# ypw0102/GDR

Hardware: AMD Instinct MI355X
Metric: queries/sec on NQ-320k (768-d) (higher is better)
Workload: dtype f32; 1 GPU; C2/ragged/prefilter: t5-base encoder 512 q/GPU + Q.D^T top-100, 320000x768 corpus; batch_per_gpu=512, global_batch=512, seq_len=40, corpus_rows=320000, dim=768, k=100, encoder_rows=ragged

## Files before the change

gdr_amd/_ffi.py:

```python
import ctypes as C
import os

_HERE = os.path.dirname(os.path.abspath(__file__))
LIB_PATH = os.environ.get("GDR_HIP_LIB") or os.path.join(_HERE, "libgdr_hip.so")

GDR_OK, GDR_EINVAL, GDR_ENOSPC, GDR_EHIP = 0, -1, -2, -3
ABI_VERSION = 9
RERANK_POSITIONS = 1
SIM_EXHAUSTIVE = 1
SIM_NO_STREAM = 2
EPI_NONE, EPI_RESIDUAL, EPI_RELU, EPI_BIAS, EPI_BIAS_RELU, EPI_BIAS_RESIDUAL, EPI_BIAS_GELU = range(7)


class GdrError(RuntimeError):
    pass


class GdrT5Dims(C.Structure):
    _fields_ = [("vocab_size", C.c_int32), ("d_model", C.c_int32), ("d_kv", C.c_int32), ("d_ff", C.c_int32),
                ("num_heads", C.c_int32), ("num_layers", C.c_int32), ("rel_buckets", C.c_int32),
                ("rel_max_distance", C.c_int32), ("eps", C.c_float)]


class GdrT5EncLayer(C.Structure):
    _fields_ = [(n, C.c_void_p) for n in ("ln_attn", "wqkv", "wo", "ln_ff", "wi", "wo_ff")]


class GdrT5EncoderWeights(C.Structure):
    _fields_ = [("dims", GdrT5Dims), ("embed", C.c_void_p), ("rel_bias", C.c_void_p), ("final_ln", C.c_void_p),
                ("layers", C.POINTER(GdrT5EncLayer))]


class GdrBertLayer(C.Structure):
    _fields_ = [(n, C.c_void_p) for n in ("wqkv", "bqkv", "wo", "bo", "ln1_w", "ln1_b", "wi", "bi", "wo2", "bo2", "ln2_w",
                                          "ln2_b")]


class GdrBertWeights(C.Structure):
    _fields_ = [("vocab_size", C.c_int32), ("d_model", C.c_int32), ("num_heads", C.c_int32), ("d_ff", C.c_int32),
                ("num_layers", C.c_int32), ("max_pos", C.c_int32), ("type_vocab", C.c_int32), ("eps", C.c_float),
                ("word_emb", C.c_void_p), ("pos_emb", C.c_void_p), ("type_emb", C.c_void_p), ("emb_ln_w", C.c_void_p),
                ("emb_ln_b", C.c_void_p), ("layers", C.POINTER(GdrBertLayer))]


class GdrTrie(C.Structure):
    _fields_ = [("child", C.c_void_p), ("eos_ok", C.c_void_p), ("n_nodes", C.c_int32), ("V", C.c_int32)]


class GdrPrefixTable(C.Structure):
    _fields_ = [("child", C.c_void_p), ("n_nodes", C.c_int32), ("V", C.c_int32), ("n_table", C.c_int32),
                ("kv", C.c_void_p), ("W", C.c_void_p), ("complete_levels", C.c_int32)]


class GdrClusterIndex(C.Structure):
    _fields_ = [("n_clusters", C.c_int32), ("key_len", C.c_int32), ("table_size", C.c_int32), ("slots", C.c_void_p),
                ("keys", C.c_void_p), ("key_lens", C.c_void_p), ("offsets", C.c_void_p), ("members", C.c_void_p)]


class GdrT5DecLayer(C.Structure):
    _fields_ = [(n, C.c_void_p) for n in ("ln_self", "wqkv", "wo", "ln_cross", "wq_c", "wkv_c", "wo_c", "ln_ff", "wi",
                                          "wo_ff")]


class GdrAdaptorLayer(C.Structure):
    _fields_ = [(n, C.c_void_p) for n in ("in_w", "in_b", "out_w", "out_b", "ln1_w", "ln1_b", "cross_const", "ln2_w",
                                          "ln2_b", "lin1_w", "lin1_b", "lin2_w", "lin2_b", "ln3_w", "ln3_b")]


class GdrT5DecoderWeights(C.Structure):
    _fields_ = [("dims", GdrT5Dims), ("out_vocab", C.c_int32), ("max_out_len", C.c_int32),
                ("adaptor_layers", C.c_int32), ("adaptor_nhead", C.c_int32), ("adaptor_ff", C.c_int32),
                ("adaptor_eps", C.c_float), ("dec_embed", C.c_void_p), ("self_rel_bias", C.c_void_p),
                ("cross_rel_bias", C.c_void_p), ("final_ln", C.c_void_p), ("layers", C.POINTER(GdrT5DecLayer)),
                ("alayers", C.POINTER(GdrAdaptorLayer)), ("head_w", C.c_void_p), ("head_e", C.c_void_p)]


_vp, _i, _i64, _sz, _f = C.c_void_p, C.c_int, C.c_int64, C.c_size_t, C.c_float
SIGNATURES = {
    "gdr_last_error": (C.c_char_p, []),
    "gdr_abi_version": (_i, []),
    "gdr_device_fault_pending": (_i, []),
    "gdr_device_fault_clear": (None, []),
    "gdr_device_fault_inject_for_tests": (None, []),
# ... 128 lines not shown
```

gdr_amd/csrc/encoder.hip:

```cpp
#include <stdlib.h>

#include "layers.h"

namespace gdr {

constexpr size_t ENC_SPLITK_BYTES = (size_t)112 << 20;
static_assert(STREAMK_BYTES <= ENC_SPLITK_BYTES, "stream-K scratch must fit the split-K region");

static int enc_streamk(char* splitk_region, StreamK* sk, hipStream_t stream) {
  sk->part = reinterpret_cast<float*>(splitk_region);
  sk->flag = reinterpret_cast<int32_t*>(splitk_region + STREAMK_PART_BYTES);
  sk->epoch = 0;
  if (hipMemsetAsync(sk->flag, 0, 512 * sizeof(int32_t), stream) != hipSuccess) {
    set_error("t5_encoder: memset of the stream-K flags failed");
    return GDR_EHIP;
  }
  return GDR_OK;
}

struct EncWs {
  size_t off_h, off_nx, off_qkv, off_ctx, off_ff, off_splitk, off_bf, total;
};

static EncWs enc_ws(const GdrT5Dims& dm, int64_t M, bool bf16 = false) {
  EncWs w{};
  const size_t inner = (size_t)dm.num_heads * dm.d_kv;
  size_t o = 0;
  w.off_h = o, o += align_up((size_t)M * dm.d_model * 4, 256);
  w.off_nx = o, o += align_up((size_t)M * dm.d_model * 4, 256);
  w.off_qkv = o, o += align_up((size_t)M * 3 * inner * 4, 256);
  w.off_ctx = o, o += align_up((size_t)M * inner * 4, 256);
  w.off_ff = o, o += align_up((size_t)M * dm.d_ff * 4, 256);
  w.off_splitk = o, o += ENC_SPLITK_BYTES;
  w.off_bf = o;
  if (bf16) o += align_up((size_t)M * (dm.d_ff > dm.d_model ? dm.d_ff : dm.d_model) * 2, 256);
  w.total = o;
  return w;
}

}

extern "C" size_t gdr_t5_encoder_workspace_bytes(const GdrT5Dims* dims, int B, int L) {
  if (!dims || B <= 0 || L <= 0) return 0;
  return gdr::enc_ws(*dims, (int64_t)B * L).total;
}

namespace gdr {
static int t5_encoder_impl(const GdrT5EncoderWeights* w, const int64_t* ids, const int64_t* mask, int B, int L,
                           float* out_hidden, float* out_pooled, void* workspace, size_t workspace_bytes, bool bf16,
                           hipStream_t stream) {
  if (B == 0) return GDR_OK;
  GDR_CHECK_ARG(w && ids && out_hidden && workspace, "t5_encoder: null pointer");
  const GdrT5Dims& dm = w->dims;
  GDR_CHECK_ARG(B > 0 && L > 0 && L <= 128, "t5_encoder: B=%d L=%d (L must be in [1,128])", B, L);
  GDR_CHECK_ARG(dm.d_model % 4 == 0 && dm.d_kv % 4 == 0 && dm.d_ff % 4 == 0, "t5_encoder: dims must be multiples of 4");
  GDR_CHECK_ARG(w->embed && w->rel_bias && w->final_ln && w->layers, "t5_encoder: null weight pointer");
  const int64_t M = (int64_t)B * L;
  const EncWs ws = enc_ws(dm, M, bf16);
  GDR_CHECK_ARG(!bf16 || (dm.d_model % 8 == 0 && dm.d_ff % 8 == 0 && (dm.num_heads * dm.d_kv) % 8 == 0),
                "t5_encoder_bf16: dims must be multiples of 8");
// ... 197 lines not shown
    const bool pooled_only = out_hidden == nullptr;
    for (int i = 0; i < dm.num_layers; ++i) {
      const GdrT5EncLayer& ly = w->layers[i];
      GDR_CHECK_ARG(ly.ln_attn && ly.wqkv && ly.wo && ly.ln_ff && ly.wi && ly.wo_ff, "t5_encoder_ragged: layer %d null weight", i);
      if ((rc = launch_rmsnorm_bf16_dev(h, ly.ln_attn, abf, rows_dev, M, d, dm.eps, stream))) return rc;
      if ((rc = lin16(abf, ly.wqkv, qkv, 3 * inner, M, rows_dev, 3 * inner, d, 0, nullptr, 1))) return rc;
      if ((rc = launch_attention(at, stream))) return rc;
      if (pooled_only && i == dm.num_layers - 1) {
        if ((rc = launch_gather_rows(static_cast<const float*>(abf), seq_off, B, inner / 2, static_cast<float*>(ctx_cls16), stream)))
          return rc;
        if ((rc = launch_gather_rows(h, seq_off, B, d, h_cls, stream))) return rc;
        if ((rc = lin16(ctx_cls16, ly.wo, h_cls, d, B, nullptr, d, inner, 0, h_cls, 0))) return rc;
        if ((rc = launch_rmsnorm_bf16(h_cls, ly.ln_ff, nx_cls16, B, d, dm.eps, stream))) return rc;
        if ((rc = lin16(nx_cls16, ly.wi, static_cast<float*>(ff_cls16), dm.d_ff, B, nullptr, dm.d_ff, d, 1, nullptr, 1))) return rc;
        if ((rc = lin16(ff_cls16, ly.wo_ff, h_cls, d, B, nullptr, d, dm.d_ff, 0, h_cls, 0))) return rc;
        return launch_rmsnorm(h_cls, w->final_ln, out_pooled, B, d, dm.eps, nullptr, 1, stream);
      }
      if ((rc = lin16(abf, ly.wo, h, d, M, rows_dev, d, inner, 0, h, 0))) return rc;
      if ((rc = launch_rmsnorm_bf16_dev(h, ly.ln_ff, abf, rows_dev, M, d, dm.eps, stream))) return rc;
      if ((rc = lin16(abf, ly.wi, ff, dm.d_ff, M, rows_dev, dm.d_ff, d, 1, nullptr, 1))) return rc;
      if ((rc = lin16(ff, ly.wo_ff, h, d, M, rows_dev, d, dm.d_ff, 0, h, 0))) return rc;
    }
    if ((rc = launch_rmsnorm_dev(h, w->final_ln, nx, rows_dev, M, d, dm.eps, stream))) return rc;
    if (out_pooled && (rc = launch_gather_rows(nx, seq_off, B, d, out_pooled, stream))) return rc;
    if (out_hidden) {
      if (hipMemsetAsync(out_hidden, 0, (size_t)M * d * sizeof(float), stream) != hipSuccess) {
        set_error("t5_encoder_ragged: memset failed");
        return GDR_EHIP;
      }
      if ((rc = launch_scatter_rows(nx, row_src, rows_dev, M, d, out_hidden, stream))) return rc;
    }
    return GDR_OK;
  }
  float* h = reinterpret_cast<float*>(base + ws.off_h);
  float* nx = reinterpret_cast<float*>(base + ws.off_nx);
  float* qkv = reinterpret_cast<float*>(base + ws.off_qkv);
  float* ctx = reinterpret_cast<float*>(base + ws.off_ctx);
  float* ff = reinterpret_cast<float*>(base + ws.off_ff);
  float* ctx_cls = reinterpret_cast<float*>(base + rw.ctx_cls);
  float* h_cls = reinterpret_cast<float*>(base + rw.h_cls);
  float* nx_cls = reinterpret_cast<float*>(base + rw.nx_cls);
  float* ff_cls = reinterpret_cast<float*>(base + rw.ff_cls);
  StreamK sk{};
  if ((rc = enc_streamk(base + ws.off_splitk, &sk, stream))) return rc;
  float* skw = reinterpret_cast<float*>(base + ws.off_splitk);
  auto linear = [&](const float* A, int64_t lda, const float* W, float* C, int64_t ldc, int N, int K, int epi,
                    const float* residual) -> int {
    if (small)
      return launch_linear_f32_ws(A, lda, W, K, C, ldc, M, N, K, epi, nullptr, residual, ldc, skw, ENC_SPLITK_BYTES, stream, &sk,
                                  rows_dev, live_rows_hint);
    return launch_linear_f32_dev(A, lda, W, K, C, ldc, M, rows_dev, N, K, epi, nullptr, residual, ldc, live_rows_hint, stream,
                                 &sk);
  };
  if ((rc = launch_embed_packed(w->embed, ids, row_src, rows_dev, M, d, dm.vocab_size, h, stream))) return rc;

  AttnArgs at{};
  at.q = qkv, at.k = qkv + inner, at.v = qkv + 2 * inner, at.out = ctx;
  at.ldq = at.ldk = at.ldv = 3 * inner, at.ldo = inner;
  at.q_bstride = at.k_bstride = at.o_bstride = L;
  at.B = B, at.H = H, at.dk = dk, at.Lq = L, at.Lk = L;
  at.q_pos0 = 0, at.scale = 1.0f;
  at.rel_bias = w->rel_bias, at.bidirectional = 1, at.num_buckets = dm.rel_buckets;
  at.lut = make_bucket_lut(dm.rel_buckets / 2, dm.rel_max_distance);
  at.key_mask = mask, at.mask_bstride = L, at.causal = 0, at.causal_neg_inf = 0;
  at.kv_rows = nullptr, at.kv_group = 1;
  at.seq_off = seq_off, at.seq_len = seq_len;

  const bool pooled_only = out_hidden == nullptr && big;
  for (int i = 0; i < dm.num_layers; ++i) {
    const GdrT5EncLayer& ly = w->layers[i];
    GDR_CHECK_ARG(ly.ln_attn && ly.wqkv && ly.wo && ly.ln_ff && ly.wi && ly.wo_ff, "t5_encoder_ragged: layer %d null weight", i);
    if ((rc = launch_rmsnorm_dev(h, ly.ln_attn, nx, rows_dev, M, d, dm.eps, stream))) return rc;
    if ((rc = linear(nx, d, ly.wqkv, qkv, 3 * inner, 3 * inner, d, GDR_EPI_NONE, nullptr))) return rc;
    if ((rc = launch_attention(at, stream))) return rc;
    if (pooled_only && i == dm.num_layers - 1) {
      if ((rc = launch_gather_rows(ctx, seq_off, B, inner, ctx_cls, stream))) return rc;
      if ((rc = launch_gather_rows(h, seq_off, B, d, h_cls, stream))) return rc;
      if ((rc = launch_linear_f32(ctx_cls, inner, ly.wo, inner, h_cls, d, B, d, inner, GDR_EPI_RESIDUAL, nullptr, h_cls, d, stream)))
        return rc;
      if ((rc = launch_rmsnorm(h_cls, ly.ln_ff, nx_cls, B, d, dm.eps, nullptr, 1, stream))) return rc;
      if ((rc = launch_linear_f32(nx_cls, d, ly.wi, d, ff_cls, dm.d_ff, B, dm.d_ff, d, GDR_EPI_RELU, nullptr, nullptr, 0, stream)))
        return rc;
      if ((rc = launch_linear_f32(ff_cls, dm.d_ff, ly.wo_ff, dm.d_ff, h_cls, d, B, d, dm.d_ff, GDR_EPI_RESIDUAL, nullptr, h_cls, d,
                                  stream)))
        return rc;
      return launch_rmsnorm(h_cls, w->final_ln, out_pooled, B, d, dm.eps, nullptr, 1, stream);
    }
    if ((rc = linear(ctx, inner, ly.wo, h, d, d, inner, GDR_EPI_RESIDUAL, h))) return rc;
    if ((rc = launch_rmsnorm_dev(h, ly.ln_ff, nx, rows_dev, M, d, dm.eps, stream))) return rc;
    if ((rc = linear(nx, d, ly.wi, ff, dm.d_ff, dm.d_ff, d, GDR_EPI_RELU, nullptr))) return rc;
    if ((rc = linear(ff, dm.d_ff, ly.wo_ff, h, d, d, dm.d_ff, GDR_EPI_RESIDUAL, h))) return rc;
  }
  if ((rc = launch_rmsnorm_dev(h, w->final_ln, nx, rows_dev, M, d, dm.eps, stream))) return rc;
  if (out_pooled && (rc = launch_gather_rows(nx, seq_off, B, d, out_pooled, stream))) return rc;
  if (out_hidden) {
    if (hipMemsetAsync(out_hidden, 0, (size_t)M * d * sizeof(float), stream) != hipSuccess) {
      set_error("t5_encoder_ragged: memset failed");
      return GDR_EHIP;
    }
    if ((rc = launch_scatter_rows(nx, row_src, rows_dev, M, d, out_hidden, stream))) return rc;
  }
  return GDR_OK;
}
}

namespace gdr {
static size_t split_ws_a_bytes(const GdrT5Dims& dm, int64_t M) {
  const int inner = dm.num_heads * dm.d_kv;
  int ld = split_row_elems(dm.d_model);
  if (split_row_elems(inner) > ld) ld = split_row_elems(inner);
  return align_up((size_t)M * ld * 2, 256);
}
static size_t split_ws_bytes(const GdrT5Dims& dm, int64_t M) {
  return split_ws_a_bytes(dm, M) + align_up((size_t)M * split_row_elems(dm.d_ff) * 2, 256);
}

static int ragged_split_impl(const GdrT5EncoderWeights* w, const int64_t* ids, const int64_t* mask, int B, int L, float* out_hidden,
                             float* out_pooled, int64_t live_rows_hint, int terms, void* workspace, size_t workspace_bytes,
                             hipStream_t stream) {
  if (B == 0) return GDR_OK;
  GDR_CHECK_ARG(terms == 6 || terms == 3 || terms == 2, "t5_encoder_split: terms must be 6 or 3 (bf16 planes) or 2 (fp16 x 2)");
  const int f16 = terms == 2 ? 1 : 0;
  GDR_CHECK_ARG(w && ids && mask && workspace && (out_hidden || out_pooled), "t5_encoder_split: null pointer");
  const GdrT5Dims& dm = w->dims;
  GDR_CHECK_ARG(B > 0 && L > 0 && L <= 128, "t5_encoder_split: B=%d L=%d (L must be in [1,128])", B, L);
  GDR_CHECK_ARG(w->embed && w->rel_bias && w->final_ln && w->layers, "t5_encoder_split: null weight pointer");
// ... 155 lines not shown
```

gdr_amd/csrc/layers.h:

```cpp
#pragma once
#include "common.h"

namespace gdr {

struct BucketLut {
  uint8_t v[128];
};
BucketLut make_bucket_lut(int nb, int max_distance);

struct AttnArgs {
  const float* q;
  const float* k;
  const float* v;
  float* out;
  void* out_bf16;
  int64_t ldq, ldk, ldv, ldo;
  int64_t q_bstride, k_bstride, o_bstride;
  int B, H, dk, Lq, Lk;
  int q_pos0;
  float scale;
  const float* rel_bias;
  int bidirectional, num_buckets;
  BucketLut lut;
  const int64_t* key_mask;
  int64_t mask_bstride;
  int causal;
  int causal_neg_inf;
  const int32_t* kv_rows;
  int kv_group;
  int q_same_pos;
  const int32_t* seq_off;
  const int32_t* seq_len;
  int qkv_bf16;
  const int64_t* b_count_dev;
  const float* q_part;
  int q_S, q_tiles_n;
  const int32_t* live;
};
int launch_attention(const AttnArgs& a, hipStream_t stream);
int launch_attention_long(const AttnArgs& a, hipStream_t stream);

int launch_embed(const float* table, const int64_t* ids, int64_t rows, int d, int vocab, float* out,
                 hipStream_t stream);
int launch_pack_plan(const int64_t* mask, int B, int L, int32_t* seq_len, int32_t* seq_off, int32_t* row_src,
                     int64_t* rows_total, hipStream_t stream);
int launch_embed_packed(const float* table, const int64_t* ids, const int32_t* row_src, const int64_t* rows_dev,
                        int64_t max_rows, int d, int vocab, float* out, hipStream_t stream);
int launch_gather_rows(const float* src, const int32_t* idx, int n, int d, float* dst, hipStream_t stream);
int launch_scatter_rows(const float* src, const int32_t* row_src, const int64_t* rows_dev, int64_t max_rows, int d,
                        float* dst, hipStream_t stream);
int launch_rmsnorm(const float* x, const float* w, float* y, int64_t rows, int d, float eps, float* pooled,
                   int pool_every, hipStream_t stream, void* y16 = nullptr);
int launch_zero_dead_rows(float* x, const int32_t* seq_len, int B, int L, int d, hipStream_t stream);
int launch_rmsnorm_dev(const float* x, const float* w, float* y, const int64_t* rows_dev, int64_t max_rows, int d, float eps,
                       hipStream_t stream, void* y16 = nullptr);
int launch_rmsnorm_planes(const float* x, const float* w, float* y, void* planes, int64_t ld, const int64_t* rows_dev, int64_t max_rows,
                          int d, float eps, hipStream_t stream, int f16x2 = 0);
int launch_rmsnorm_bf16(const float* x, const float* w, void* y_bf16, int64_t rows, int d, float eps, hipStream_t stream);
int launch_rmsnorm_bf16_dev(const float* x, const float* w, void* y_bf16, const int64_t* rows_dev, int64_t max_rows, int d,
                            float eps, hipStream_t stream);
int launch_layernorm(const float* x, const float* w, const float* b, float* y, int64_t rows, int d, float eps,
                     const float* addv, hipStream_t stream, void* y16 = nullptr, int f16x2_ld = 0);
int launch_layernorm_dev(const float* x, const float* w, const float* b, float* y, const int64_t* rows_dev, int64_t max_rows,
                         int d, float eps, const float* addv, hipStream_t stream, void* y16 = nullptr, int f16x2_ld = 0);
int launch_layernorm2(const float* x, const float* w1, const float* b1, const float* w2, const float* b2, const float* addv, float* y,
                      const int64_t* rows_dev, int64_t max_rows, int d, float eps, hipStream_t stream, void* y16 = nullptr);

}
```

gdr_amd/csrc/layers.hip:

```cpp
#include <math.h>

#include <stdlib.h>

#include "layers.h"

namespace gdr {

BucketLut make_bucket_lut(int nb, int max_distance) {
  BucketLut l;
  const int max_exact = nb / 2;
  for (int n = 0; n < 128; ++n) {
    int b;
    if (n < max_exact) {
      b = n;
    } else {
      const float v = logf((float)n / (float)max_exact) / (float)log((double)max_distance / max_exact) *
                      (float)(nb - max_exact);
      b = max_exact + (int)v;
      if (b > nb - 1) b = nb - 1;
    }
    l.v[n] = (uint8_t)b;
  }
  return l;
}
// ... 63 lines not shown
    __syncthreads();
  }
  if (tid == 0) {
    seq_off[B] = carry;
    *rows_total = carry;
  }
}

__global__ __launch_bounds__(256) void pack_rows_kernel(int B, int L, const int32_t* __restrict__ seq_len,
                                                        const int32_t* __restrict__ seq_off, int32_t* __restrict__ row_src) {
  const int b = blockIdx.x * 4 + (threadIdx.x >> 6), lane = threadIdx.x & 63;
  if (b >= B) return;
  const int o = seq_off[b], n = seq_len[b];
  for (int j = lane; j < n; j += 64) row_src[o + j] = b * L + j;
}

int launch_pack_plan(const int64_t* mask, int B, int L, int32_t* seq_len, int32_t* seq_off, int32_t* row_src,
                     int64_t* rows_total, hipStream_t stream) {
  GDR_CHECK_ARG(mask && seq_len && seq_off && row_src && rows_total, "pack_plan: null pointer");
  GDR_CHECK_ARG((int64_t)B * L < 0x7fffffffLL, "pack_plan: batch too large");
  const unsigned g = (unsigned)((B + 3) / 4);
  hipLaunchKernelGGL(pack_len_kernel, dim3(g), dim3(256), 0, stream, mask, B, L, seq_len);
  GDR_CHECK_LAUNCH("pack_len_kernel");
  hipLaunchKernelGGL(pack_scan_kernel, dim3(1), dim3(1024), 0, stream, B, seq_len, seq_off, rows_total);
  GDR_CHECK_LAUNCH("pack_scan_kernel");
  hipLaunchKernelGGL(pack_rows_kernel, dim3(g), dim3(256), 0, stream, B, L, seq_len, seq_off, row_src);
  GDR_CHECK_LAUNCH("pack_rows_kernel");
  return GDR_OK;
}

__global__ __launch_bounds__(256) void embed_packed_kernel(const float* __restrict__ table, const int64_t* __restrict__ ids,
                                                           const int32_t* __restrict__ row_src,
                                                           const int64_t* __restrict__ rows_dev, int d4, int vocab,
                                                           float* __restrict__ out) {
  const int64_t row = (int64_t)blockIdx.x * 4 + (threadIdx.x >> 6);
  if (row >= *rows_dev) return;
  int64_t id = ids[row_src[row]];
  id = id < 0 ? 0 : (id >= vocab ? vocab - 1 : id);
  const float4* src = reinterpret_cast<const float4*>(table) + id * d4;
  float4* dst = reinterpret_cast<float4*>(out) + row * d4;
  for (int c = threadIdx.x & 63; c < d4; c += 64) dst[c] = src[c];
}

int launch_embed_packed(const float* table, const int64_t* ids, const int32_t* row_src, const int64_t* rows_dev,
                        int64_t max_rows, int d, int vocab, float* out, hipStream_t stream) {
  GDR_CHECK_ARG(d % 4 == 0, "embed: d %% 4 != 0");
  if (max_rows == 0) return GDR_OK;
  hipLaunchKernelGGL(embed_packed_kernel, dim3((unsigned)((max_rows + 3) / 4)), dim3(256), 0, stream, table, ids, row_src,
                     rows_dev, d / 4, vocab, out);
  GDR_CHECK_LAUNCH("embed_packed_kernel");
  return GDR_OK;
}

template <bool SCATTER>
__global__ __launch_bounds__(256) void move_rows_kernel(const float* __restrict__ src, const int32_t* __restrict__ map,
                                                        int64_t n, const int64_t* __restrict__ n_dev, int d4,
                                                        float* __restrict__ dst) {
  const int64_t i = (int64_t)blockIdx.x * 4 + (threadIdx.x >> 6);
  if (n_dev) n = *n_dev;
  if (i >= n) return;
  const int64_t m = map[i];
  const float4* s = reinterpret_cast<const float4*>(src) + (SCATTER ? i : m) * d4;
  float4* o = reinterpret_cast<float4*>(dst) + (SCATTER ? m : i) * d4;
  for (int c = threadIdx.x & 63; c < d4; c += 64) o[c] = s[c];
}

int launch_gather_rows(const float* src, const int32_t* idx, int n, int d, float* dst, hipStream_t stream) {
  GDR_CHECK_ARG(d % 4 == 0, "gather_rows: d %% 4 != 0");
  if (n == 0) return GDR_OK;
  hipLaunchKernelGGL(move_rows_kernel<false>, dim3((unsigned)((n + 3) / 4)), dim3(256), 0, stream, src, idx, (int64_t)n,
                     (const int64_t*)nullptr, d / 4, dst);
  GDR_CHECK_LAUNCH("gather_rows");
  return GDR_OK;
}

int launch_scatter_rows(const float* src, const int32_t* row_src, const int64_t* rows_dev, int64_t max_rows, int d,
                        float* dst, hipStream_t stream) {
  GDR_CHECK_ARG(d % 4 == 0, "scatter_rows: d %% 4 != 0");
  if (max_rows == 0) return GDR_OK;
  hipLaunchKernelGGL(move_rows_kernel<true>, dim3((unsigned)((max_rows + 3) / 4)), dim3(256), 0, stream, src, row_src,
                     max_rows, rows_dev, d / 4, dst);
  GDR_CHECK_LAUNCH("scatter_rows");
  return GDR_OK;
}

__global__ __launch_bounds__(256) void zero_dead_rows_kernel(float* __restrict__ x, const int32_t* __restrict__ seq_len,
                                                             int64_t rows, int L, int d4) {
  const int64_t row = (int64_t)blockIdx.x * 4 + (threadIdx.x >> 6);
  if (row >= rows) return;
  const int b = (int)(row / L), j = (int)(row - (int64_t)b * L);
  if (j < seq_len[b]) return;
  float4* o = reinterpret_cast<float4*>(x) + row * d4;
  for (int c = threadIdx.x & 63; c < d4; c += 64) o[c] = make_float4(0.f, 0.f, 0.f, 0.f);
}

int launch_zero_dead_rows(float* x, const int32_t* seq_len, int B, int L, int d, hipStream_t stream) {
  GDR_CHECK_ARG(d % 4 == 0, "zero_dead_rows: d %% 4 != 0");
  const int64_t rows = (int64_t)B * L;
  if (rows == 0) return GDR_OK;
  hipLaunchKernelGGL(zero_dead_rows_kernel, dim3((unsigned)((rows + 3) / 4)), dim3(256), 0, stream, x, seq_len, rows, L, d / 4);
  GDR_CHECK_LAUNCH("zero_dead_rows_kernel");
  return GDR_OK;
}

__device__ __forceinline__ uint2 pack_bf16x4(float a, float b, float c, float d) {
  union {
    __bf16 h[4];
    uint2 u;
  } o;
  o.h[0] = (__bf16)a, o.h[1] = (__bf16)b, o.h[2] = (__bf16)c, o.h[3] = (__bf16)d;
  return o.u;
}

template <bool BF16OUT>
__global__ __launch_bounds__(256) void rmsnorm_kernel(const float* __restrict__ x, const float* __restrict__ w,
                                                      float* __restrict__ y, int64_t rows, int d4, float eps,
                                                      float* __restrict__ pooled, int pool_every,
                                                      const int64_t* __restrict__ rows_dev, uint2* __restrict__ y16 = nullptr,
                                                      int planes_ld = 0) {
  const int64_t row = (int64_t)blockIdx.x * 4 + (threadIdx.x >> 6);
  if (rows_dev) rows = *rows_dev;
  if (row >= rows) return;
  const int lane = threadIdx.x & 63;
  const float4* xr = reinterpret_cast<const float4*>(x) + row * d4;
  constexpr int MAXC = 8;
  const bool in_regs = d4 <= 64 * MAXC;
  float4 xv[MAXC];
  float ss = 0.f;
  if (in_regs) {
#pragma unroll
    for (int i = 0; i < MAXC; ++i) {
      const int c = lane + 64 * i;
      xv[i] = c < d4 ? xr[c] : make_float4(0.f, 0.f, 0.f, 0.f);
    }
// ... 1399 lines not shown
```

gdr_amd/ops.py:

```python
import ctypes as C
import math

import torch

from . import _ffi
from ._ffi import check, lib, ptr, stream_ptr


def _need_cuda(*ts):
    for t in ts:
        if t is not None and not t.is_cuda:
            raise _ffi.GdrError("gdr_amd ops need CUDA (ROCm) tensors; there is no CPU path")


def _f32c(t):
    if t.dtype != torch.float32:
        raise _ffi.GdrError(f"expected float32 tensor, got {t.dtype}")
    return t if t.is_contiguous() else t.contiguous()


def linear(a, w, epilogue=_ffi.EPI_NONE, bias=None, residual=None, out=None, splitk_ws=None):
    _need_cuda(a, w, bias, residual)
    K = a.shape[-1]
    a2 = _f32c(a).view(-1, K)
    w = _f32c(w)
    M, N = a2.shape[0], w.shape[0]
    if out is None:
        out = torch.empty((M, N), dtype=torch.float32, device=a.device)
    res2 = None
    if residual is not None:
        res2 = _f32c(residual).view(-1, N)
    if splitk_ws is not None:
        check(lib().gdr_linear_f32_splitk(ptr(a2), K, ptr(w), w.shape[1], ptr(out), N, M, N, K, epilogue,
                                          ptr(_f32c(bias)) if bias is not None else None, ptr(res2), N, ptr(splitk_ws),
                                          splitk_ws.numel() * splitk_ws.element_size(), stream_ptr()),
              "gdr_linear_f32_splitk")
        return out.view(*a.shape[:-1], N)
    check(lib().gdr_linear_f32(ptr(a2), K, ptr(w), w.shape[1], ptr(out), N, M, N, K, epilogue,
                               ptr(_f32c(bias)) if bias is not None else None, ptr(res2), N, stream_ptr()),
          "gdr_linear_f32")
    return out.view(*a.shape[:-1], N)


def linear_bf16(a, w, epilogue=_ffi.EPI_NONE, bias=None, residual=None, out=None):
    _need_cuda(a, w, bias, residual)
    a = (a if a.dtype == torch.bfloat16 else to_bf16(a)).contiguous()
    w = (w if w.dtype == torch.bfloat16 else to_bf16(w)).contiguous()
    K = a.shape[-1]
    a2 = a.view(-1, K)
    M, N = a2.shape[0], w.shape[0]
    if out is None:
        out = torch.empty((M, N), dtype=torch.float32, device=a.device)
    res2 = _f32c(residual).view(-1, N) if residual is not None else None
    check(lib().gdr_linear_bf16(ptr(a2), K, ptr(w), w.shape[1], ptr(out), N, M, N, K, epilogue,
# ... 522 lines not shown

def kmeans_partition(rows, labels, node_offsets, k, work=None, workspace=None):
    _kmeans_check("kmeans_partition", None, rows, node_offsets, k)
    _need_cuda(labels, work)
    n, S = rows.numel(), node_offsets.numel() - 1
    if labels.dtype != torch.int32 or labels.numel() != n:
        raise _ffi.GdrError("kmeans_partition: labels must be int32[n]")
    rows, labels, node_offsets = rows.contiguous(), labels.contiguous(), node_offsets.contiguous()
    if work is None:
        work = kmeans_worklist(node_offsets, lib().gdr_kmeans_partition_tile())
    if work.dtype != torch.int32 or work.dim() != 2 or work.shape[1] != 2 or work.shape[0] == 0:
        raise _ffi.GdrError("kmeans_partition: work must be int32[n_work, 2]")
    dev = rows.device
    out_rows = torch.empty((n,), dtype=torch.int32, device=dev)
    child = torch.empty((S * k + 1,), dtype=torch.int32, device=dev)
    status = torch.empty((1,), dtype=torch.int32, device=dev)
    need = lib().gdr_kmeans_partition_workspace_bytes(work.shape[0], k)
    ws = (workspace or Workspace(dev)).get(need)
    check(lib().gdr_kmeans_partition(ptr(rows), ptr(labels), n, ptr(node_offsets), S, k, ptr(work.contiguous()), work.shape[0],
                                     ptr(out_rows), ptr(child), ptr(status), ptr(ws), ws.numel(), stream_ptr()),
          "gdr_kmeans_partition")
    return out_rows, child, status


def kmeans_centroids(D, child_offsets, rows, workspace=None):
    _need_cuda(D, child_offsets, rows)
    if D.dtype != torch.float32:
        raise _ffi.GdrError(f"kmeans_centroids: the corpus must be float32, got {D.dtype} (a bf16 corpus is not supported)")
    D = _f32c(D)
    if child_offsets.dtype != torch.int32 or rows.dtype != torch.int32:
        raise _ffi.GdrError("kmeans_centroids: expected int32 child_offsets / rows")
    N, d = D.shape
    C_, n = child_offsets.numel() - 1, rows.numel()
    if C_ < 1 or n < 1:
        raise _ffi.GdrError("kmeans_centroids: empty level")
    cent = torch.empty((C_, d), dtype=torch.float32, device=D.device)
    counts = torch.empty((C_,), dtype=torch.int32, device=D.device)
    need = lib().gdr_kmeans_centroids_workspace_bytes(n, d)
    ws = (workspace or Workspace(D.device)).get(need)
    check(lib().gdr_kmeans_centroids(ptr(D), N, d, ptr(child_offsets.contiguous()), ptr(rows.contiguous()), n, C_, ptr(cent),
                                     ptr(counts), ptr(ws), ws.numel(), stream_ptr()), "gdr_kmeans_centroids")
    return cent, counts


def relative_bucket_table(bidirectional, num_buckets, max_distance, qlen, klen):
    buf = (C.c_int32 * (qlen * klen))()
    check(lib().gdr_t5_relative_bucket_table(int(bidirectional), num_buckets, max_distance, qlen, klen, buf),
          "gdr_t5_relative_bucket_table")
    return torch.tensor(list(buf), dtype=torch.int32).view(qlen, klen)


class T5EncoderHandle:

    def __init__(self, cfg, sd, device, prefix="encoder.", dtype=torch.float32, split=False):
        if dtype not in (torch.float32, torch.bfloat16):
            raise ValueError("T5EncoderHandle: dtype must be float32 or bfloat16")
        if split and dtype != torch.float32:
            raise ValueError("T5EncoderHandle: split=True is a form of the float32 mode")
        if split not in (False, True, 0, 2, 3, 6):
            raise ValueError("T5EncoderHandle: split must be False, True (= 6 terms), 3 / 6 (bf16 planes) or 2 (fp16 x 2)")
        self.cfg, self.device, self.dtype, self.split = cfg, device, dtype, (6 if split is True else int(split))
        keep = []

        def dev(t):
            t = t.detach().to(device=device, dtype=torch.float32).contiguous()
            keep.append(t)
            return t

        def lin(t):
            t = dev(t)
            if dtype == torch.bfloat16:
                keep.pop()
                t = to_bf16(t)
                keep.append(t)
            elif split:
                keep.pop()
                t = split_f16x2(t) if int(split) == 2 else split_bf16x3(t)
                keep.append(t)
            return t

        self.embed = dev(sd["shared.weight"] if "shared.weight" in sd else sd[prefix + "embed_tokens.weight"])
        self.rel_bias = dev(sd[prefix + "block.0.layer.0.SelfAttention.relative_attention_bias.weight"])
        self.final_ln = dev(sd[prefix + "final_layer_norm.weight"])
        nl = cfg.num_layers
        self._layers = (_ffi.GdrT5EncLayer * nl)()
        for i in range(nl):
            p = f"{prefix}block.{i}.layer."
            wqkv = lin(torch.cat([sd[p + "0.SelfAttention.q.weight"], sd[p + "0.SelfAttention.k.weight"],
                                  sd[p + "0.SelfAttention.v.weight"]], dim=0))
            L = self._layers[i]
            L.ln_attn = dev(sd[p + "0.layer_norm.weight"]).data_ptr()
            L.wqkv = wqkv.data_ptr()
            L.wo = lin(sd[p + "0.SelfAttention.o.weight"]).data_ptr()
            L.ln_ff = dev(sd[p + "1.layer_norm.weight"]).data_ptr()
            L.wi = lin(sd[p + "1.DenseReluDense.wi.weight"]).data_ptr()
            L.wo_ff = lin(sd[p + "1.DenseReluDense.wo.weight"]).data_ptr()
        self._keep = keep
        self.dims = _ffi.GdrT5Dims(cfg.vocab_size, cfg.d_model, cfg.d_kv, cfg.d_ff, cfg.num_heads, nl,
                                   cfg.relative_attention_num_buckets, cfg.relative_attention_max_distance,
                                   cfg.layer_norm_epsilon)
        self.struct = _ffi.GdrT5EncoderWeights(self.dims, self.embed.data_ptr(), self.rel_bias.data_ptr(),
                                               self.final_ln.data_ptr(), self._layers)
        self.ws = Workspace(device)

    def forward(self, input_ids, attention_mask=None, want_pooled=True, want_hidden=True, ragged=False,
                live_rows_hint=-1):
        _need_cuda(input_ids, attention_mask)
        ids = input_ids.to(torch.int64).contiguous()
        B, L = ids.shape
        if attention_mask is None:
            attention_mask = torch.ones_like(ids)
        mask = attention_mask.to(torch.int64).contiguous()
        bf = self.dtype == torch.bfloat16
        if not (want_hidden or want_pooled):
            raise ValueError("T5EncoderHandle.forward: nothing requested")
        d = self.cfg.d_model
        pooled = torch.empty((B, d), dtype=torch.float32, device=ids.device) if want_pooled else None
        if self.split:
            if not ragged:
                raise _ffi.GdrError("T5EncoderHandle(split=True): the split form exists for the ragged forward only")
            need = lib().gdr_t5_encoder_split_workspace_bytes(C.byref(self.dims), B, L)
            ws = self.ws.get(need)
            out = torch.empty((B, L, d), dtype=torch.float32, device=ids.device) if want_hidden else None
            check(lib().gdr_t5_encoder_forward_ragged_split(C.byref(self.struct), ptr(ids), ptr(mask), B, L, ptr(out), ptr(pooled),
                                                            int(live_rows_hint), self.split, ptr(ws), ws.numel(), stream_ptr()),
                  "gdr_t5_encoder_forward_ragged_split")
            return out, pooled
        if ragged:
            need = lib().gdr_t5_encoder_ragged_workspace_bytes(C.byref(self.dims), B, L)
            ws = self.ws.get(need)
            out = torch.empty((B, L, d), dtype=torch.float32, device=ids.device) if want_hidden else None
            rfn = lib().gdr_t5_encoder_forward_ragged_bf16 if bf else lib().gdr_t5_encoder_forward_ragged
            check(rfn(C.byref(self.struct), ptr(ids), ptr(mask), B, L, ptr(out), ptr(pooled), int(live_rows_hint), ptr(ws),
                      ws.numel(), stream_ptr()), "gdr_t5_encoder_forward_ragged")
            return out, pooled
        need = (lib().gdr_t5_encoder_bf16_workspace_bytes if bf else lib().gdr_t5_encoder_workspace_bytes)(
            C.byref(self.dims), B, L)
        ws = self.ws.get(need)
        out = torch.empty((B, L, d), dtype=torch.float32, device=ids.device)
        fn = lib().gdr_t5_encoder_forward_bf16 if bf else lib().gdr_t5_encoder_forward
        check(fn(C.byref(self.struct), ptr(ids), ptr(mask), B, L, ptr(out), ptr(pooled), ptr(ws), ws.numel(),
                 stream_ptr()), "gdr_t5_encoder_forward")
        return (out if want_hidden else None), pooled


BERT_MAX_LEN = 512
ATTN_LONG_QUERY_BLOCK = 128
ATTN_LONG_KEY_BLOCK = 64


class BertEncoderHandle:

    def __init__(self, bcfg, sd, device, prefix="ctx_encoder.bert_model.", dtype=torch.float32, split=False):
        if dtype not in (torch.float32, torch.bfloat16):
            raise ValueError("BertEncoderHandle: dtype must be float32 or bfloat16")
        if split and dtype != torch.float32:
# ... 322 lines not shown
```

include/gdr_hip.h:

```cpp
#ifndef GDR_HIP_H
#define GDR_HIP_H

#include <stddef.h>
#include <stdint.h>

#ifdef __cplusplus
extern "C" {
#endif

#define GDR_OK 0
#define GDR_EINVAL (-1)
#define GDR_ENOSPC (-2)
#define GDR_EHIP (-3)

const char* gdr_last_error(void);
int gdr_abi_version(void);
int64_t gdr_launch_count(void);

int gdr_prof_enable(int max_events);
int gdr_prof_collect(int64_t* launches, double* total_ms, double* total_work);
void gdr_prof_gate(int on);

enum {
  GDR_EPI_NONE = 0,
// ... 4 lines not shown
  GDR_EPI_BIAS_RESIDUAL = 5,
  GDR_EPI_BIAS_GELU = 6
};
int gdr_linear_f32(const float* A, int64_t lda, const float* W, int64_t ldw, float* C, int64_t ldc,
                   int64_t M, int N, int K, int epilogue, const float* bias, const float* residual,
                   int64_t ldr, void* stream);
int gdr_linear_f32_splitk(const float* A, int64_t lda, const float* W, int64_t ldw, float* C, int64_t ldc,
                          int64_t M, int N, int K, int epilogue, const float* bias, const float* residual,
                          int64_t ldr, void* workspace, size_t workspace_bytes, void* stream);

#define GDR_F32_FORM_TILES 1
#define GDR_F32_FORM_PERSISTENT 2
#define GDR_F32_FORM_SMALL 3
#define GDR_F32_FORM_SMALL_SPLITK 4
#define GDR_F32_FORM_SPLITK 5
#define GDR_F32_FORM_STREAMK_256 6
#define GDR_F32_FORM_STREAMK_TAIL 7
int gdr_linear_f32_form(int64_t M, int N, int K, size_t workspace_bytes);

int gdr_linear_bf16(const void* A, int64_t lda, const void* W, int64_t ldw, float* C, int64_t ldc, int64_t M, int N,
                    int K, int epilogue, const float* bias, const float* residual, int64_t ldr, void* stream);
int gdr_split_row_elems(int K, int terms);
int gdr_split_f32_bf16x3(const float* in, void* out_planes, int64_t rows, int K, int64_t ld_out, void* stream);
int gdr_split_f32_f16x2(const float* in, void* out_planes, int64_t rows, int K, int64_t ld_out, void* stream);
int gdr_linear_split_bf16(const void* A3, int64_t lda, const void* W3, int64_t ldw, float* C, int64_t ldc, int64_t M, int N, int K,
                          int terms, int epilogue, const float* bias, const float* residual, int64_t ldr, void* stream);
int gdr_linear_bf16_tile_form(int64_t M, int N, int K, int epilogue);

int gdr_t5_layer_norm(const float* x, const float* w, float* y, int64_t rows, int d, float eps, void* stream);

int gdr_l2_normalize(const float* x, float* y, int64_t rows, int d, float eps, void* stream);

typedef struct {
  int32_t vocab_size, d_model, d_kv, d_ff, num_heads, num_layers;
  int32_t rel_buckets, rel_max_distance;
  float eps;
} GdrT5Dims;

typedef struct {
  const float* ln_attn;
  const float* wqkv;
  const float* wo;
  const float* ln_ff;
  const float* wi;
  const float* wo_ff;
} GdrT5EncLayer;

typedef struct {
  GdrT5Dims dims;
  const float* embed;
  const float* rel_bias;
  const float* final_ln;
  const GdrT5EncLayer* layers;
} GdrT5EncoderWeights;

size_t gdr_t5_encoder_workspace_bytes(const GdrT5Dims* dims, int B, int L);
int gdr_t5_encoder_forward(const GdrT5EncoderWeights* w, const int64_t* ids, const int64_t* mask, int B, int L,
                           float* out_hidden, float* out_pooled, void* workspace, size_t workspace_bytes,
                           void* stream);

size_t gdr_t5_encoder_ragged_workspace_bytes(const GdrT5Dims* dims, int B, int L);
int gdr_t5_encoder_forward_ragged(const GdrT5EncoderWeights* w, const int64_t* ids, const int64_t* mask, int B, int L,
                                  float* out_hidden, float* out_pooled, int64_t live_rows_hint, void* workspace,
                                  size_t workspace_bytes, void* stream);

int gdr_t5_encoder_forward_ragged_bf16(const GdrT5EncoderWeights* w, const int64_t* ids, const int64_t* mask, int B, int L,
                                       float* out_hidden, float* out_pooled, int64_t live_rows_hint, void* workspace,
                                       size_t workspace_bytes, void* stream);
size_t gdr_t5_encoder_split_workspace_bytes(const GdrT5Dims* dims, int B, int L);
int gdr_t5_encoder_forward_ragged_split(const GdrT5EncoderWeights* w, const int64_t* ids, const int64_t* mask, int B, int L,
                                        float* out_hidden, float* out_pooled, int64_t live_rows_hint, int terms, void* workspace,
                                        size_t workspace_bytes, void* stream);

size_t gdr_t5_encoder_bf16_workspace_bytes(const GdrT5Dims* dims, int B, int L);
int gdr_t5_encoder_forward_bf16(const GdrT5EncoderWeights* w, const int64_t* ids, const int64_t* mask, int B, int L,
                                float* out_hidden, float* out_pooled, void* workspace, size_t workspace_bytes,
                                void* stream);

#define GDR_SIM_EXHAUSTIVE 1
#define GDR_SIM_NO_STREAM 2
size_t gdr_sim_topk_workspace_bytes(int B, int64_t N, int d, int k, int flags);
int gdr_sim_topk(const float* Q, int B, const float* D, int64_t N, int d, int k, int32_t idx_offset,
                 float* out_val, int32_t* out_idx, int32_t* status, int flags, void* workspace,
                 size_t workspace_bytes, void* stream);

int gdr_sim_topk_bf16(const void* Q, int B, const void* D, int64_t N, int d, int k, int32_t idx_offset,
                      float* out_val, int32_t* out_idx, int32_t* status, int flags, void* workspace,
                      size_t workspace_bytes, void* stream);
size_t gdr_sim_topk_prefilter_workspace_bytes(int B, int64_t N, int d, int k);
int gdr_sim_topk_prefilter(const float* Q, int B, const float* D, const void* D_bf16, float dnorm_max, int64_t N, int d, int k,
                           int32_t idx_offset, float* out_val, int32_t* out_idx, int32_t* status, void* workspace,
                           size_t workspace_bytes, void* stream);
int gdr_row_norm2_max(const float* D, int64_t N, int d, float* out_dev, void* stream);
int gdr_cast_f32_bf16(const float* in, void* out_bf16, int64_t n, void* stream);

int gdr_topk_merge(const float* vals, const int32_t* idx, int G, int B, int k, float* out_val, int32_t* out_idx,
                   void* stream);
int gdr_topk_pack(const float* vals, const int32_t* idx, const int32_t* status, int B, int k, void* pairs, void* stream);
int gdr_topk_merge_packed(const void* pairs, int G, int B, int k, float* out_val, int32_t* out_idx,
                          int32_t* out_status, void* stream);

#define GDR_RERANK_POSITIONS 1
size_t gdr_rerank_workspace_bytes(int B, int max_cand);
int gdr_rerank_topk(const float* q, const float* D, int d, const int32_t* cand_offsets, const int32_t* cand_ids,
                    const float* beam_scores, int B, int R, const float* alphas, int A, int k, int func,
                    float* out_val, int32_t* out_idx, int max_cand, int cand_stride, int32_t doc_lo, int32_t doc_hi,
// ... 177 lines not shown
```

Measured before the change: 30490 queries/s.

## Precompute layer-0 QKV per vocab token and compute last-layer Q only for CLS rows

Layer 0's RMSNorm and QKV projection depend only on the token id, so a vocab-sized table of projected QKV rows is built at weight load. The embedding kernel then copies both the hidden row and the QKV row, which removes the first layer's norm and QKV GEMM. In the pooled-only final layer, K and V are still projected for all rows, but Q is projected only for the gathered CLS rows and scattered back into the QKV buffer. The cost is a vocab by 3*inner fp32 table (about 32k x 2304 floats) that must be refreshed whenever weights change, plus extra gather and scatter launches.

New measurement: 31230 queries/s (median of 6 runs). 2.4% higher.

```diff
diff --git a/gdr_amd/_ffi.py b/gdr_amd/_ffi.py
--- a/gdr_amd/_ffi.py
+++ b/gdr_amd/_ffi.py
@@ -28,7 +28,7 @@
 
 class GdrT5EncoderWeights(C.Structure):
     _fields_ = [("dims", GdrT5Dims), ("embed", C.c_void_p), ("rel_bias", C.c_void_p), ("final_ln", C.c_void_p),
-                ("layers", C.POINTER(GdrT5EncLayer))]
+                ("layers", C.POINTER(GdrT5EncLayer)), ("qkv0_table", C.c_void_p)]
 
 
 class GdrBertLayer(C.Structure):
diff --git a/gdr_amd/csrc/encoder.hip b/gdr_amd/csrc/encoder.hip
--- a/gdr_amd/csrc/encoder.hip
+++ b/gdr_amd/csrc/encoder.hip
@@ -6,6 +6,7 @@
 
 constexpr size_t ENC_SPLITK_BYTES = (size_t)112 << 20;
 static_assert(STREAMK_BYTES <= ENC_SPLITK_BYTES, "stream-K scratch must fit the split-K region");
+constexpr bool ENC_LAST_Q_CLS_DEFAULT = true;
 
 static int enc_streamk(char* splitk_region, StreamK* sk, hipStream_t stream) {
   sk->part = reinterpret_cast<float*>(splitk_region);
@@ -309,7 +310,13 @@
     return launch_linear_f32_dev(A, lda, W, K, C, ldc, M, rows_dev, N, K, epi, nullptr, residual, ldc, live_rows_hint, stream,
                                  &sk);
   };
-  if ((rc = launch_embed_packed(w->embed, ids, row_src, rows_dev, M, d, dm.vocab_size, h, stream))) return rc;
+  const float* qkv0 = big ? w->qkv0_table : nullptr;
+  GDR_CHECK_ARG(!qkv0 || (((uintptr_t)qkv0) & 15) == 0, "t5_encoder_ragged: qkv0_table must be 16-byte aligned");
+  if (qkv0)
+    rc = launch_embed_packed2(w->embed, qkv0, ids, row_src, rows_dev, M, d, 3 * inner, dm.vocab_size, h, qkv, stream);
+  else
+    rc = launch_embed_packed(w->embed, ids, row_src, rows_dev, M, d, dm.vocab_size, h, stream);
+  if (rc) return rc;
 
   AttnArgs at{};
   at.q = qkv, at.k = qkv + inner, at.v = qkv + 2 * inner, at.out = ctx;
@@ -324,11 +331,25 @@
   at.seq_off = seq_off, at.seq_len = seq_len;
 
   const bool pooled_only = out_hidden == nullptr && big;
+  static const bool last_q_cls_on = [] {
+    const char* e = getenv("GDR_ENC_LAST_Q_CLS");
+    return e ? atoi(e) != 0 : ENC_LAST_Q_CLS_DEFAULT;
+  }();
   for (int i = 0; i < dm.num_layers; ++i) {
     const GdrT5EncLayer& ly = w->layers[i];
     GDR_CHECK_ARG(ly.ln_attn && ly.wqkv && ly.wo && ly.ln_ff && ly.wi && ly.wo_ff, "t5_encoder_ragged: layer %d null weight", i);
-    if ((rc = launch_rmsnorm_dev(h, ly.ln_attn, nx, rows_dev, M, d, dm.eps, stream))) return rc;
-    if ((rc = linear(nx, d, ly.wqkv, qkv, 3 * inner, 3 * inner, d, GDR_EPI_NONE, nullptr))) return rc;
+    if (i == 0 && qkv0) {
+    } else if (pooled_only && i == dm.num_layers - 1 && last_q_cls_on) {
+      if ((rc = launch_rmsnorm_dev(h, ly.ln_attn, nx, rows_dev, M, d, dm.eps, stream))) return rc;
+      if ((rc = linear(nx, d, ly.wqkv + (size_t)inner * d, qkv + inner, 3 * inner, 2 * inner, d, GDR_EPI_NONE, nullptr))) return rc;
+      if ((rc = launch_gather_rows(nx, seq_off, B, d, nx_cls, stream))) return rc;
+      if ((rc = launch_linear_f32(nx_cls, d, ly.wqkv, d, ctx_cls, inner, B, inner, d, GDR_EPI_NONE, nullptr, nullptr, 0, stream)))
+        return rc;
+      if ((rc = launch_scatter_rows_strided(ctx_cls, seq_off, B, inner, qkv, 3 * inner, stream))) return rc;
+    } else {
+      if ((rc = launch_rmsnorm_dev(h, ly.ln_attn, nx, rows_dev, M, d, dm.eps, stream))) return rc;
+      if ((rc = linear(nx, d, ly.wqkv, qkv, 3 * inner, 3 * inner, d, GDR_EPI_NONE, nullptr))) return rc;
+    }
     if ((rc = launch_attention(at, stream))) return rc;
     if (pooled_only && i == dm.num_layers - 1) {
       if ((rc = launch_gather_rows(ctx, seq_off, B, inner, ctx_cls, stream))) return rc;
diff --git a/gdr_amd/csrc/layers.h b/gdr_amd/csrc/layers.h
--- a/gdr_amd/csrc/layers.h
+++ b/gdr_amd/csrc/layers.h
@@ -46,7 +46,11 @@
                      int64_t* rows_total, hipStream_t stream);
 int launch_embed_packed(const float* table, const int64_t* ids, const int32_t* row_src, const int64_t* rows_dev,
                         int64_t max_rows, int d, int vocab, float* out, hipStream_t stream);
+int launch_embed_packed2(const float* table, const float* table2, const int64_t* ids, const int32_t* row_src,
+                         const int64_t* rows_dev, int64_t max_rows, int d, int e, int vocab, float* out, float* out2,
+                         hipStream_t stream);
 int launch_gather_rows(const float* src, const int32_t* idx, int n, int d, float* dst, hipStream_t stream);
+int launch_scatter_rows_strided(const float* src, const int32_t* idx, int n, int d, float* dst, int64_t ldd, hipStream_t stream);
 int launch_scatter_rows(const float* src, const int32_t* row_src, const int64_t* rows_dev, int64_t max_rows, int d,
                         float* dst, hipStream_t stream);
 int launch_rmsnorm(const float* x, const float* w, float* y, int64_t rows, int d, float eps, float* pooled,
diff --git a/gdr_amd/csrc/layers.hip b/gdr_amd/csrc/layers.hip
--- a/gdr_amd/csrc/layers.hip
+++ b/gdr_amd/csrc/layers.hip
@@ -139,16 +139,43 @@
   return GDR_OK;
 }
 
+__global__ __launch_bounds__(256) void embed_packed2_kernel(const float* __restrict__ table, const float* __restrict__ table2,
+                                                            const int64_t* __restrict__ ids, const int32_t* __restrict__ row_src,
+                                                            const int64_t* __restrict__ rows_dev, int d4, int e4, int vocab,
+                                                            float* __restrict__ out, float* __restrict__ out2) {
+  const int64_t row = (int64_t)blockIdx.x * 4 + (threadIdx.x >> 6);
+  if (row >= *rows_dev) return;
+  int64_t id = ids[row_src[row]];
+  id = id < 0 ? 0 : (id >= vocab ? vocab - 1 : id);
+  const float4* src2 = reinterpret_cast<const float4*>(table2) + id * e4;
+  float4* dst2 = reinterpret_cast<float4*>(out2) + row * e4;
+  for (int c = threadIdx.x & 63; c < e4; c += 64) dst2[c] = src2[c];
+  const float4* src = reinterpret_cast<const float4*>(table) + id * d4;
+  float4* dst = reinterpret_cast<float4*>(out) + row * d4;
+  for (int c = threadIdx.x & 63; c < d4; c += 64) dst[c] = src[c];
+}
+
+int launch_embed_packed2(const float* table, const float* table2, const int64_t* ids, const int32_t* row_src,
+                         const int64_t* rows_dev, int64_t max_rows, int d, int e, int vocab, float* out, float* out2,
+                         hipStream_t stream) {
+  GDR_CHECK_ARG(d % 4 == 0 && e % 4 == 0, "embed: d %% 4 != 0");
+  if (max_rows == 0) return GDR_OK;
+  hipLaunchKernelGGL(embed_packed2_kernel, dim3((unsigned)((max_rows + 3) / 4)), dim3(256), 0, stream, table, table2, ids,
+                     row_src, rows_dev, d / 4, e / 4, vocab, out, out2);
+  GDR_CHECK_LAUNCH("embed_packed2_kernel");
+  return GDR_OK;
+}
+
 template <bool SCATTER>
 __global__ __launch_bounds__(256) void move_rows_kernel(const float* __restrict__ src, const int32_t* __restrict__ map,
                                                         int64_t n, const int64_t* __restrict__ n_dev, int d4,
-                                                        float* __restrict__ dst) {
+                                                        float* __restrict__ dst, int64_t dst_ld4) {
   const int64_t i = (int64_t)blockIdx.x * 4 + (threadIdx.x >> 6);
   if (n_dev) n = *n_dev;
   if (i >= n) return;
   const int64_t m = map[i];
   const float4* s = reinterpret_cast<const float4*>(src) + (SCATTER ? i : m) * d4;
-  float4* o = reinterpret_cast<float4*>(dst) + (SCATTER ? m : i) * d4;
+  float4* o = reinterpret_cast<float4*>(dst) + (SCATTER ? m : i) * dst_ld4;
   for (int c = threadIdx.x & 63; c < d4; c += 64) o[c] = s[c];
 }
 
@@ -156,8 +183,17 @@
   GDR_CHECK_ARG(d % 4 == 0, "gather_rows: d %% 4 != 0");
   if (n == 0) return GDR_OK;
   hipLaunchKernelGGL(move_rows_kernel<false>, dim3((unsigned)((n + 3) / 4)), dim3(256), 0, stream, src, idx, (int64_t)n,
-                     (const int64_t*)nullptr, d / 4, dst);
+                     (const int64_t*)nullptr, d / 4, dst, (int64_t)(d / 4));
   GDR_CHECK_LAUNCH("gather_rows");
+  return GDR_OK;
+}
+
+int launch_scatter_rows_strided(const float* src, const int32_t* idx, int n, int d, float* dst, int64_t ldd, hipStream_t stream) {
+  GDR_CHECK_ARG(d % 4 == 0 && ldd % 4 == 0 && ldd >= d && ((uintptr_t)dst & 15) == 0, "scatter_rows: bad row width / stride / alignment");
+  if (n == 0) return GDR_OK;
+  hipLaunchKernelGGL(move_rows_kernel<true>, dim3((unsigned)((n + 3) / 4)), dim3(256), 0, stream, src, idx, (int64_t)n,
+                     (const int64_t*)nullptr, d / 4, dst, ldd / 4);
+  GDR_CHECK_LAUNCH("scatter_rows_strided");
   return GDR_OK;
 }
 
@@ -166,7 +202,7 @@
   GDR_CHECK_ARG(d % 4 == 0, "scatter_rows: d %% 4 != 0");
   if (max_rows == 0) return GDR_OK;
   hipLaunchKernelGGL(move_rows_kernel<true>, dim3((unsigned)((max_rows + 3) / 4)), dim3(256), 0, stream, src, row_src,
-                     max_rows, rows_dev, d / 4, dst);
+                     max_rows, rows_dev, d / 4, dst, (int64_t)(d / 4));
   GDR_CHECK_LAUNCH("scatter_rows");
   return GDR_OK;
 }
diff --git a/gdr_amd/ops.py b/gdr_amd/ops.py
--- a/gdr_amd/ops.py
+++ b/gdr_amd/ops.py
@@ -1,5 +1,6 @@
 import ctypes as C
 import math
+import os
 
 import torch
 
@@ -628,7 +629,7 @@
 
 class T5EncoderHandle:
 
-    def __init__(self, cfg, sd, device, prefix="encoder.", dtype=torch.float32, split=False):
+    def __init__(self, cfg, sd, device, prefix="encoder.", dtype=torch.float32, split=False, token_table=None):
         if dtype not in (torch.float32, torch.bfloat16):
             raise ValueError("T5EncoderHandle: dtype must be float32 or bfloat16")
         if split and dtype != torch.float32:
@@ -665,7 +666,10 @@
             wqkv = lin(torch.cat([sd[p + "0.SelfAttention.q.weight"], sd[p + "0.SelfAttention.k.weight"],
                                   sd[p + "0.SelfAttention.v.weight"]], dim=0))
             L = self._layers[i]
-            L.ln_attn = dev(sd[p + "0.layer_norm.weight"]).data_ptr()
+            ln_attn = dev(sd[p + "0.layer_norm.weight"])
+            if i == 0:
+                self._ln0, self._wqkv0 = ln_attn, wqkv
+            L.ln_attn = ln_attn.data_ptr()
             L.wqkv = wqkv.data_ptr()
             L.wo = lin(sd[p + "0.SelfAttention.o.weight"]).data_ptr()
             L.ln_ff = dev(sd[p + "1.layer_norm.weight"]).data_ptr()
@@ -678,6 +682,27 @@
         self.struct = _ffi.GdrT5EncoderWeights(self.dims, self.embed.data_ptr(), self.rel_bias.data_ptr(),
                                                self.final_ln.data_ptr(), self._layers)
         self.ws = Workspace(device)
+        if token_table is None:
+            token_table = os.environ.get("GDR_ENC_TOKEN_TABLE", "1") != "0"
+        inner = cfg.num_heads * cfg.d_kv
+        packs = cfg.d_kv == 64 and cfg.d_model % 32 == 0 and cfg.d_ff % 32 == 0 and inner % 32 == 0
+        self.token_table = None
+        if token_table and dtype == torch.float32 and not split and packs:
+            self.token_table = torch.empty((cfg.vocab_size, 3 * inner), dtype=torch.float32, device=device)
+            self.refresh_token_table()
+            self.struct.qkv0_table = self.token_table.data_ptr()
+
+    @property
+    def token_table_bytes(self):
+        return 0 if self.token_table is None else self.token_table.numel() * 4
+
+    def refresh_token_table(self, chunk=4096):
+        if self.token_table is None:
+            return self
+        for s in range(0, self.cfg.vocab_size, chunk):
+            e = min(s + chunk, self.cfg.vocab_size)
+            linear(t5_layer_norm(self.embed[s:e], self._ln0, self.cfg.layer_norm_epsilon), self._wqkv0, out=self.token_table[s:e])
+        return self
 
     def forward(self, input_ids, attention_mask=None, want_pooled=True, want_hidden=True, ragged=False,
                 live_rows_hint=-1):
diff --git a/include/gdr_hip.h b/include/gdr_hip.h
--- a/include/gdr_hip.h
+++ b/include/gdr_hip.h
@@ -80,6 +80,7 @@
   const float* rel_bias;
   const float* final_ln;
   const GdrT5EncLayer* layers;
+  const float* qkv0_table;
 } GdrT5EncoderWeights;
 
 size_t gdr_t5_encoder_workspace_bytes(const GdrT5Dims* dims, int B, int L);
```
